# cherubicXN/neat

Measured on AMD Instinct MI355X. Metric: ray-samples/s (train step) on ABC-neat-a, higher is better.
Workload: dtype bf16; 1 GPU; C2: abc-neat-a networks, 1024 rays x 128 samples per GPU, depth samples given, train step = forward + loss + backward + Adam; rays_per_gpu=1024, samples_per_ray=128, global_rays=1024, parallelism=dp1, weights=synthetic 'rough' (seed 42), launch=hip graph replay, the whole step one launch (forward + loss + backward + Adam)

## Files before the change

neat_amd/csrc/kernels_bf16.hpp:

```cpp
#pragma once
#include "kernels.hpp"
#include "bf16_common.hpp"

namespace neat {

__device__ __forceinline__ size_t oct_index(int f, int p, int ldp) { return ((size_t)(f >> 3) * ldp + p) * 8 + (f & 7); }

struct SegH { const void* p; int rows; int bf16; };

struct LayerArgsH {
  SegH in[2];
  int Kpad;
  const uint4* Wp;
  const float* bias;
  int bias_rot, bias_n;
  int N, NT;
  int ldp;
  void* out0; void* out1;
  int out0_bf16, out1_bf16, n_split, accumulate;
  const u16* aux0; const u16* aux1;
  const u16* padfill_oct;
  const float* padfill; int padfill_rows;
};

// ... 753 lines not shown
      eh[3 + 6 * k + c] = f * __cosf(xc * f) * gc;
      eh[6 + 6 * k + c] = -f * __sinf(xc * f) * gc;
      f *= 2.0f;
    }
  }
  eh[39] = 0.0f; ev[39] = 0.0f;
#pragma unroll
  for (int j = 0; j < 39; ++j) { a.Eh[(size_t)j * ldp + p] = eh[j]; ev[j] = a.E[(size_t)j * ldp + p]; }
  auto octet = [](const float (&v)[40], int r0) {
    float t[8];
#pragma unroll
    for (int e = 0; e < 8; ++e) t[e] = (r0 + e < 39) ? v[r0 + e] : 0.0f;
    return make_uint4(pack2(t[0], t[1]), pack2(t[2], t[3]), pack2(t[4], t[5]), pack2(t[6], t[7]));
  };
#pragma unroll
  for (int o = 0; o < 5; ++o) {
    reinterpret_cast<uint4*>(a.Ebf)[(size_t)o * ldp + p] = octet(ev, 8 * o);
    reinterpret_cast<uint4*>(a.Ehbf)[(size_t)o * ldp + p] = octet(eh, 8 * o);
  }
#pragma unroll
  for (int o = 0; o < 4; ++o) {
    reinterpret_cast<uint4*>(a.Ebf4)[(size_t)o * ldp + p] = octet(ev, 7 + 8 * o);
    reinterpret_cast<uint4*>(a.Ehbf4)[(size_t)o * ldp + p] = octet(eh, 7 + 8 * o);
  }
}

#ifndef NEAT_W3_ABLATE
#define NEAT_W3_ABLATE 0
#endif
constexpr int W3T = 512, W3P = 32, W3NS = 4;
template <int NCB> struct W3Cfg {
  static constexpr int QA = 8, QB = 2 * NCB;
  static constexpr int STAGE = (QA + QB) * 2048;
  static constexpr int LDS = W3NS * STAGE;
  static constexpr int QPW = NCB == 5 ? 3 : 2;
  static constexpr int G = 2 * QPW;
};
constexpr int W3_STAGE = W3Cfg<4>::STAGE;
constexpr int W3_LDS_BYTES = W3Cfg<4>::LDS;
constexpr int W3_SLOTS = 12;
struct WgradArgsH3 {
  const unsigned short* A[W3_SLOTS]; const unsigned short* B[W3_SLOTS]; int rowsA[W3_SLOTS];
  const unsigned short* B2[W3_SLOTS];
  int splitB, octsB;
  int npairs, N, K, P, ldp, chunk;
  float* partial; size_t row_stride, split_stride; int col_off, bias_col;
  int nt_loads;
  int interleave;
  int nprob; size_t prob_stride;
};
typedef short v4s16 __attribute__((ext_vector_type(4)));

template <int NCB>
__global__ __launch_bounds__(W3T, 2) void wgrad_kernel_h3(WgradArgsH3 a) {
  typedef W3Cfg<NCB> C;
  extern __shared__ __attribute__((aligned(16))) unsigned char w3lds[];
  typedef __attribute__((address_space(3))) void* lds_ptr;
  typedef __attribute__((address_space(3))) v4s16* lds_v4;
  typedef const __attribute__((address_space(1))) void* gbl_ptr;
  const int tid = threadIdx.x, lane = tid & 63, wave = tid >> 6;
  const int wr = (wave >> 1) * 64, wc = (wave & 1) * 32 * NCB;
  const int nsplit = gridDim.y;
  const int pstep = a.interleave ? nsplit * W3P : W3P;
  const int pbeg = a.interleave ? blockIdx.y * W3P : blockIdx.y * a.chunk;
  const int pend = a.interleave ? a.P : min(a.P, pbeg + a.chunk);
  const int nsteps = a.interleave ? ((a.P + W3P - 1) / W3P - (int)blockIdx.y + nsplit - 1) / nsplit : (pend - pbeg + W3P - 1) / W3P;
  const int prob = a.nprob > 1 ? (int)blockIdx.x : 0;
  const int T = nsteps * a.npairs;
  bool liveR[2], liveC[NCB];
#pragma unroll
  for (int i = 0; i < 2; ++i) liveR[i] = wr + 32 * i < a.N;
#pragma unroll
  for (int j = 0; j < NCB; ++j) liveC[j] = wc + 32 * j < a.K;
  f32x16 acc[2][NCB];
#pragma unroll
  for (int i = 0; i < 2; ++i)
#pragma unroll
    for (int j = 0; j < NCB; ++j)
#pragma unroll
      for (int r = 0; r < 16; ++r) acc[i][j][r] = 0.0f;
  float rsum[2] = {0.0f, 0.0f};

  const int dl_oct = lane & 3, dl_pt = lane >> 2;
  const unsigned lds_base = (unsigned)(size_t)(lds_ptr)w3lds;
  const unsigned short* opbase[2][C::QPW]; const unsigned short* opbase2[2]; int opmax[2][C::QPW]; int opq[C::QPW]; bool opB[C::QPW];
#pragma unroll
  for (int hq = 0; hq < C::QPW; ++hq) {
    const int g = min(C::QPW * wave + hq, C::QA + C::QB - 1);
    opB[hq] = g >= C::QA; opq[hq] = opB[hq] ? g - C::QA : g;
  }
#pragma unroll
  for (int q = 0; q < 2; ++q) {
    const int idx = prob * a.npairs + q;
    const unsigned short* pA = a.A[0]; const unsigned short* pB = a.B[0]; const unsigned short* p2 = a.B2[0];
    int rA = a.rowsA[0];
#pragma unroll
    for (int k = 1; k < W3_SLOTS; ++k)
      if (idx == k) { pA = a.A[k]; pB = a.B[k]; p2 = a.B2[k]; rA = a.rowsA[k]; }
    opbase2[q] = p2;
#pragma unroll
    for (int hq = 0; hq < C::QPW; ++hq) { opbase[q][hq] = opB[hq] ? pB : pA; opmax[q][hq] = opB[hq] ? a.octsB - 1 : (rA + 7) / 8 - 1; }
  }
  auto issue = [&](int tau) {
    const int q = tau >= nsteps ? 1 : 0;
    const int st = tau - q * nsteps;
    if (NEAT_W3_ABLATE == 4) return;
    const unsigned short* base2 = q ? opbase2[1] : opbase2[0];
    const unsigned stage = lds_base + (tau % W3NS) * C::STAGE;
#pragma unroll
    for (int hq = 0; hq < C::QPW; ++hq) {
      const unsigned short* base = q ? opbase[1][hq] : opbase[0][hq];
      const int maxoct = q ? opmax[1][hq] : opmax[0][hq];
      const int oct = min(4 * opq[hq] + dl_oct, maxoct);
      const bool second = opB[hq] && oct >= a.splitB;
      const uint4* seg = reinterpret_cast<const uint4*>(second ? base2 : base) + (size_t)(second ? oct - a.splitB : oct) * a.ldp;
      const int g = min(C::QPW * wave + hq, C::QA + C::QB - 1);
#ifndef NEAT_W3_SKIP_SURPLUS
#define NEAT_W3_SKIP_SURPLUS 1
#endif
      if constexpr (NEAT_W3_SKIP_SURPLUS && 8 * C::QPW > C::QA + C::QB) { if (C::QPW * wave + hq >= C::QA + C::QB) continue; }
// ... 38 lines not shown
        if (NEAT_W3_ABLATE == 2) { av[i] = make_uint4(lane, tau, i, s2); continue; }
        const unsigned char* ap = slot + ((wr >> 5) + i) * 2048 + s2 * 1024 + frag_off;
        const v4s16 lo = __builtin_amdgcn_ds_read_tr16_b64_v4i16((lds_v4)(ap));
        const v4s16 hi = __builtin_amdgcn_ds_read_tr16_b64_v4i16((lds_v4)(ap + 256));
        av[i] = make_uint4(((const unsigned*)&lo)[0], ((const unsigned*)&lo)[1], ((const unsigned*)&hi)[0], ((const unsigned*)&hi)[1]);
      }
#pragma unroll
      for (int j = 0; j < NCB; ++j) {
        if (NEAT_W3_ABLATE == 2) { bv[j] = make_uint4(lane, tau, j, s2); continue; }
        const unsigned char* bp = slot + C::QA * 2048 + ((wc >> 5) + j) * 2048 + s2 * 1024 + frag_off;
        const v4s16 lo = __builtin_amdgcn_ds_read_tr16_b64_v4i16((lds_v4)(bp));
        const v4s16 hi = __builtin_amdgcn_ds_read_tr16_b64_v4i16((lds_v4)(bp + 256));
        bv[j] = make_uint4(((const unsigned*)&lo)[0], ((const unsigned*)&lo)[1], ((const unsigned*)&hi)[0], ((const unsigned*)&hi)[1]);
      }
      if (tail) {
        const int p0 = pb + 16 * s2 + 8 * (G >> 1);
        auto mask4 = [&](uint4& v) {
          unsigned w4[4] = {v.x, v.y, v.z, v.w};
#pragma unroll
          for (int e = 0; e < 4; ++e) {
            const bool k0 = p0 + 2 * e < pend, k1 = p0 + 2 * e + 1 < pend;
            w4[e] = (k0 ? (w4[e] & 0x0000FFFFu) : 0u) | (k1 ? (w4[e] & 0xFFFF0000u) : 0u);
          }
          v = make_uint4(w4[0], w4[1], w4[2], w4[3]);
        };
#pragma unroll
        for (int i = 0; i < 2; ++i) mask4(av[i]);
#pragma unroll
        for (int j = 0; j < NCB; ++j) mask4(bv[j]);
      }
      if (bias_now) {
#pragma unroll
        for (int i = 0; i < 2; ++i) {
          const unsigned w4[4] = {av[i].x, av[i].y, av[i].z, av[i].w};
          float t = rsum[i];
#pragma unroll
          for (int e = 0; e < 4; ++e) { t += bf_lo(w4[e]); t += bf_hi(w4[e]); }
          asm volatile("" : "+v"(t));
          rsum[i] = t;
        }
      }
#pragma unroll
      for (int i = 0; i < 2; ++i) {
        if (!liveR[i]) continue;
#pragma unroll
        for (int j = 0; j < NCB; ++j)
          if (liveC[j]) {
            if (NEAT_W3_ABLATE == 1) { asm volatile("" :: "v"(av[i].x), "v"(av[i].w), "v"(bv[j].x), "v"(bv[j].w)); continue; }
            acc[i][j] = NEAT_MFMA16(*reinterpret_cast<bf16x8*>(&av[i]), *reinterpret_cast<bf16x8*>(&bv[j]), acc[i][j], 0, 0, 0);
          }
      }
    }
  }
  float* dstp = a.partial + (size_t)prob * a.prob_stride + (size_t)blockIdx.y * a.split_stride;
  auto put = [&](float* q, float v) {
    if (NEAT_W3_ABLATE == 3 && v != 123.0f) return;
    *q = v;
  };
#pragma unroll
  for (int i = 0; i < 2; ++i) {
    if (!liveR[i]) continue;
#pragma unroll
    for (int r = 0; r < 16; ++r) {
      const int n = wr + 32 * i + (r & 3) + 8 * (r >> 2) + 4 * (lane >> 5);
      if (n >= a.N) continue;
#pragma unroll
      for (int j = 0; j < NCB; ++j) {
        const int k = wc + 32 * j + (lane & 31);
        if (liveC[j] && k < a.K) put(dstp + (size_t)n * a.row_stride + a.col_off + k, acc[i][j][r]);
      }
    }
  }
  if (do_bias) {
#pragma unroll
    for (int i = 0; i < 2; ++i) {
      float v = rsum[i];
      v += __shfl_xor(v, 32);
      const int n = wr + 32 * i + (lane & 31);
      if (lane < 32 && n < a.N) put(dstp + (size_t)n * a.row_stride + a.bias_col, v);
    }
  }
}

struct PackDesc2 {
  int layer, transpose, N, K, Kpad, NT;
  int s0, s0p, off0, off1;
  int rot;
  float scale; int offset; int blk0; int bf16;
  int lo;
};
constexpr int MAXPACKS2 = 48;
struct PackArgs2 { NetPtrs net; const float* rowscale; int row_off[NLAYERS + 1]; PackDesc2 d[MAXPACKS2]; int npacks; float* out; };

__device__ __forceinline__ float packed_weight(const PackDesc2& d, const float* v, const float* rs, int O, int I, int n, int k) {
  if (!v || n >= d.N || k >= d.K) return 0.0f;
  const int po = d.transpose ? k : n;
  const int pj = d.transpose ? n : k;
  if (po >= O) return 0.0f;
  const int o = (po + d.rot) % O;
  int i;
  if (pj < d.s0p) { if (pj >= d.s0) return 0.0f; i = d.off0 + pj; }
  else { i = d.off1 + (pj - d.s0p); if (pj - d.s0p >= I - d.s0) return 0.0f; }
  if (i >= I) return 0.0f;
  return v[(size_t)o * I + i] * rs[o] * d.scale;
}

__global__ __launch_bounds__(WG) void pack_kernel2(PackArgs2 a) {
  int pk = 0;
  while (pk + 1 < a.npacks && (int)blockIdx.x >= a.d[pk + 1].blk0) ++pk;
  const PackDesc2 d = a.d[pk];
  const int nt = blockIdx.x - d.blk0;
  const int O = a.net.O[d.layer], I = a.net.I[d.layer];
  const float* v = a.net.v[d.layer];
  const float* rs = a.rowscale + a.row_off[d.layer];
  if (d.bf16) {
    const int KS = d.Kpad >> 4;
    uint4* out = reinterpret_cast<uint4*>(a.out + d.offset) + (size_t)nt * KS * 64;
    for (int e = blockIdx.y * WG + threadIdx.x; e < KS * 64; e += WG * gridDim.y) {
      const int s = e >> 6, ln = e & 63;
      const int n = nt * 32 + (ln & 31), kb = 16 * s + 8 * (ln >> 5);
      float w[8];
#pragma unroll
      for (int t = 0; t < 8; ++t) w[t] = packed_weight(d, v, rs, O, I, n, kb + t);
      if (d.lo) {
#pragma unroll
        for (int t = 0; t < 8; ++t) w[t] -= bf2f(f2bf(w[t]));
      }
      out[e] = make_uint4(pack2(w[0], w[1]), pack2(w[2], w[3]), pack2(w[4], w[5]), pack2(w[6], w[7]));
    }
  } else {
    const int KS = d.Kpad >> 1;
    float* out = a.out + d.offset + (size_t)nt * KS * 64;
    for (int e = blockIdx.y * WG + threadIdx.x; e < KS * 64; e += WG * gridDim.y) {
      const int s = e >> 6, ln = e & 63;
// ... 78 lines not shown
```

neat_amd/csrc/neat_net.hip:

```cpp
#include <mutex>
#include <unordered_map>
#if defined(NEAT_HALF) && NEAT_HALF
#define neat neat_f16
#include "f16_symbols.h"
#endif
#include "kernels_bf16.hpp"
#include "kernels_dw.hpp"
#include "fused_launch.hpp"
#include "../../include/neat_hip.h"
#include <algorithm>
#include <initializer_list>
#include <utility>
#include <math.h>
#include <stdio.h>
#include <stdlib.h>
#include <vector>

using namespace neat;

namespace {

constexpr int L_REND = 9, L_ATTR = 14;
const int kO[NLAYERS] = {256, 256, 256, 217, 256, 256, 256, 256, 257, 256, 256, 256, 256, 3, 256, 256, 256, 256, 6};
const int kI[NLAYERS] = {39, 256, 256, 256, 256, 256, 256, 256, 256, 289, 256, 256, 256, 256, 265, 256, 256, 256, 256};
// ... 111 lines not shown
  s->flops = flops; s->bytes = bytes; s->cls = cls;
  hipEventRecord(s->e0, st);
  return s;
}
inline void prof_end(hipStream_t st, ProfSlot* s) { if (s) hipEventRecord(s->e1, st); }

template <int EPI> hipError_t launch_layer_f(hipStream_t st, const LayerArgs& a, int ntiles_p) {
  NEAT_TRY(lds_limit<&layer_kernel<EPI>>(96 * 1024));
  size_t lds = (size_t)a.Kpad * BM * sizeof(float);
  if (a.NT <= 2 && lds < 32768) lds = 32768;
  hipLaunchKernelGGL(layer_kernel<EPI>, dim3(ntiles_p), dim3(WG), lds, st, a);
  return hipGetLastError();
}
int g_wgrad_h3 = 1;
int g_pt_bf16 = 2;

template <int EPI, int PT, bool OBF> hipError_t launch_layer_h_pt(hipStream_t st, const LayerArgsH& a) {
  NEAT_TRY((lds_limit<&layer_kernel_h<EPI, PT, OBF>>(96 * 1024)));
  constexpr int BMT = 32 * PT;
  size_t lds = (size_t)(a.Kpad / 8) * BMT * 16;
  const size_t red = (size_t)4 * PT * 16 * 64 * 4;
  if (a.NT <= 2 && lds < red) lds = red;
  hipLaunchKernelGGL((layer_kernel_h<EPI, PT, OBF>), dim3(a.ldp / BMT), dim3(WG), lds, st, a);
  return hipGetLastError();
}
template <int EPI> hipError_t launch_layer_h(hipStream_t st, const LayerArgsH& a, int) {
  if (a.out0_bf16) return g_pt_bf16 == 4 ? launch_layer_h_pt<EPI, 4, true>(st, a) : launch_layer_h_pt<EPI, 2, true>(st, a);
  return launch_layer_h_pt<EPI, 2, false>(st, a);
}
int g_wgrad_batch = -1;
inline int wgrad_batch_size(int ldp) {
  if (g_wgrad_batch >= 0) return g_wgrad_batch;
  return ldp <= 200000 ? 3 : (ldp <= 400000 ? 2 : 0);
}
int g_wreduce_direct = 2;
int g_head_chain = 2;
int g_fused_adj = 1;
int g_layer_ws = 1;
constexpr int WS_GRID = 256;
constexpr int DW_MAXGRID = 256;
inline int dw_slots(int ldp) {
  const int nt = ldp / WSP;
  return nt < DW_MAXGRID ? (nt > 0 ? nt : 1) : DW_MAXGRID;
}
inline int dw_grid(int ldp) {
  const int nt = ldp / WSP;
  return nt < DW_MAXGRID ? nt : DW_MAXGRID;
}
int g_ws_aux_nt = 15;
int g_ws_wide_store = 1;
const int* g_gate = nullptr; int g_gate_value = 0;
int g_ws_interleave = 1;
int g_wgrad_narrow = 1;
int g_dw_ablate = 0;
int g_dw_fused = 1;
constexpr int DW_MIN_POINTS = 49152;
constexpr int DW8_XBLOCKS = 512;
int g_dw_lin8 = 1;
int g_chain_pp = 1;
constexpr int DW_NSUB = 16;
int g_dw_segments = 1;
template <int EPI, bool FULL> hipError_t launch_layer_wsdw(hipStream_t st, const LayerArgsDW* d0, int n = 1) {
  NEAT_TRY((lds_limit<&layer_kernel_wsdw<EPI, FULL>>(WsCfg<EPI, 16>::LDS + DW_XLDS)));
  if (n < 1 || n > DW_MAXSEG || (n > 1 && !(FULL && EPI != EPI_BWD8))) return hipErrorInvalidValue;
  LayerArgsDWSeg seg{};
  seg.n = n;
  for (int i = 0; i < n; ++i) {
    LayerArgsDW& d = seg.l[i];
    d = d0[i];
    d.w.ntiles = d.w.ldp / WSP;
    d.w.aux_nt = (g_ws_aux_nt & 3) | ((g_ws_aux_nt >> 1) & 28);
    d.ablate = g_dw_ablate;
    if (FULL && (d.w.N != 256 || d.rowsA != 256)) return hipErrorInvalidValue;
    if (d.w.ldp != d0[0].w.ldp) return hipErrorInvalidValue;
  }
  hipLaunchKernelGGL((layer_kernel_wsdw<EPI, FULL>), dim3(dw_grid(seg.l[0].w.ldp)), dim3(WST), (WsCfg<EPI, 16>::LDS + DW_XLDS), st, seg);
  return hipGetLastError();
}
template <int EPI, bool FULL> hipError_t launch_layer_wsdw(hipStream_t st, const LayerArgsDW& d0) { return launch_layer_wsdw<EPI, FULL>(st, &d0, 1); }
template <int EPI, int KS = 16, bool OUTF = false> hipError_t launch_layer_ws(hipStream_t st, const LayerArgsWS& a0) {
  NEAT_TRY((lds_limit<&layer_kernel_ws<EPI, KS, OUTF>>(WsCfg<EPI, KS>::LDS)));
  LayerArgsWS a = a0;
  a.ntiles = a.ldp / WSP;
  a.per_wg = (a.ntiles + WS_GRID - 1) / WS_GRID;
  int grid = (a.ntiles + a.per_wg - 1) / a.per_wg;
  a.tile_stride = 1;
  a.wide_store = g_ws_wide_store;
  a.aux_nt = (g_ws_aux_nt & 3) | ((g_ws_aux_nt >> 1) & 28);
  a.xcd_major = g_ws_interleave == 2;
  if (g_ws_interleave) { grid = a.ntiles < WS_GRID ? a.ntiles : WS_GRID; a.tile_stride = grid; }
  hipLaunchKernelGGL((layer_kernel_ws<EPI, KS, OUTF>), dim3(grid), dim3(WST), (WsCfg<EPI, KS>::LDS), st, a);
  return hipGetLastError();
}
inline int ws_shape(int epi, const LayerArgsH& a) {
  if (!g_layer_ws) return 0;
  const bool seg1 = a.in[1].rows != 0;
  if (!a.in[0].bf16 || a.accumulate || (a.bias && a.bias_rot != 0)) return 0;
  if (a.padfill) {
    return (epi == EPI_TAN && a.padfill_oct && a.padfill_rows == 7 && a.N == 217 && a.Kpad == 256 && !seg1 && a.in[0].rows == 256 &&
            a.out0_bf16 && a.out1 && a.out1_bf16 && a.n_split >= a.N && !a.bias) ? 5 : 0;
  }
  if (a.Kpad == 320) {
    return (epi == EPI_RELU && seg1 && a.in[1].bf16 && a.in[0].rows == 256 && a.in[1].rows <= 64 && a.out0_bf16 && a.N == 256 &&
            a.n_split >= a.N && !a.out1) ? 4 : 0;
  }
  if (a.Kpad == 64 && !seg1) {
// ... 133 lines not shown
    a.out0 = out0.p; a.out1 = out1.p; a.out0_bf16 = out0.bf16; a.out1_bf16 = out1.bf16;
    a.n_split = n_split; a.accumulate = accumulate;
    a.aux0 = reinterpret_cast<const u16*>(aux0.p); a.aux1 = reinterpret_cast<const u16*>(aux1.p);
    a.padfill = padfill; a.padfill_rows = padfill_rows; a.padfill_oct = reinterpret_cast<const u16*>(padfill_oct.p);
    if ((aux0.p && !aux0.bf16) || (aux1.p && !aux1.bf16) || (out1.p && (out1.bf16 != (epi == EPI_TAN)))) return hipErrorInvalidValue;
    const int shape = ws_shape(epi, a);
    e = shape ? dispatch_ws(c.st, epi, a, shape) : dispatch_h(c.st, epi, a, c.ldp / BMH);
  }
  prof_end(c.st, ps);
  dbg_sync(c.st, "layer pid/epi/N", pid, epi, N);
  return e;
}

hipError_t layer_ws(const Ctx& c, int pid, int epi, Arr in0, int N, Arr out0, Arr aux0 = Arr{}, Arr aux1 = Arr{},
                    const float* srow = nullptr, const float* wrow = nullptr, const float* wrow_scale = nullptr,
                    const float* rho_num = nullptr, const float* rho_den = nullptr) {
  const PackDesc2& d = c.L().d[pid];
  if (!c.prec || !in0.bf16 || !out0.bf16 || N > 256 || N > d.N || d.Kpad < 256) return hipErrorInvalidValue;
  LayerArgsWS a{};
  a.in = reinterpret_cast<const u16*>(in0.p); a.Wp = reinterpret_cast<const uint4*>(c.packed + d.offset);
  a.aux0 = reinterpret_cast<const u16*>(aux0.p); a.aux1 = reinterpret_cast<const u16*>(aux1.p);
  a.out0 = reinterpret_cast<u16*>(out0.p);
  a.srow = srow; a.wrow = wrow; a.wrow_scale = wrow_scale; a.rho_num = rho_num; a.rho_den = rho_den;
  a.N = N; a.in_octs = 32; a.ldp = c.ldp; a.kstride = d.Kpad / 16;
  a.split_oct = 32; a.n_split = 1 << 30;
  const double P = (double)c.P;
  const double bytes = 256 * P * 2.0 + N * P * 2.0 * (1 + (aux0.p ? 1 : 0) + (aux1.p ? 1 : 0)) + (srow ? P * 4.0 : 0.0) + N * 256 * 2.0;
  ProfSlot* ps = prof_begin(c.st, 0, 2.0 * N * 256 * P, bytes);
  hipError_t e = dispatch_ws_args(c.st, epi, a);
  prof_end(c.st, ps);
  dbg_sync(c.st, "layer_ws pid/epi/N", pid, epi, N);
  return e;
}

inline dim3 grid1(int n, int b = 256) { return dim3((n + b - 1) / b); }

struct SdfWs {
  float *x, *E, *sdfraw, *sdf, *mask, *g, *e0, *es, *Eh, *gh, *abar8, *ones, *partial;
  Arr featc;
  Arr Ebf, Ebf4, Ehbf, Ehbf4;
  Arr h[9], feat, u[8], vh[9], m[8];
  Arr hlo[9], featlo;
  float *dwp, *dwscale, *dwbias;
  size_t total;
};
constexpr int DW_JOBS = 15;
constexpr int WSPLIT = 128;
constexpr int WLDN = 384, WLDK = 384;
constexpr int W2SPLIT = 256;
constexpr int W2LDN = 288, W2LDK = 320;
constexpr int W2_LDS_BYTES = 2 * 256 * HLD + 8 * 8 * 64 * 16;
constexpr int WGROUPS = 8;
constexpr size_t WSTAGE_FLOATS = (size_t)WGROUPS * WREDUCE_BATCH * 256 * 264;
constexpr size_t WPARTIAL_FLOATS = (size_t)W2SPLIT * W2LDN * W2LDK + WSTAGE_FLOATS;

SdfWs sdf_ws(float* base, int ldp, int mode, int prec, int hx3 = 0) {
  SdfWs w{};
  size_t off = 0;
  auto take = [&](int rows) { float* p = base ? base + off : nullptr; off += (size_t)rows * ldp; return p; };
  auto big = [&](int rows) { Arr a; a.p = take(rows); a.bf16 = prec; return a; };
  w.x = take(3); w.E = take(PE_ROWS + 1); w.sdf = take(1); w.mask = take(1); w.g = take(3); w.sdfraw = take(1);
  if (mode == 0) {
    Arr a = big(256), b = big(256);
    for (int l = 1; l <= 8; ++l) w.h[l] = (l & 1) ? a : b;
  } else if (mode == 2) {
    for (int l = 1; l <= 8; ++l) w.h[l] = big(256);
    if (prec) w.feat = big(256);
    else { float* out8 = take(257); w.sdfraw = out8; w.feat = F(out8 + ldp); }
    Arr a = big(256), b = big(256);
    for (int l = 0; l < 8; ++l) w.u[l] = (l & 1) ? a : b;
    w.e0 = take(PE_ROWS); w.es = take(PE_ROWS);
  } else {
    for (int l = 1; l <= 8; ++l) w.h[l] = big(256);
    if (prec) w.feat = big(256);
    else { float* out8 = take(257); w.sdfraw = out8; w.feat = F(out8 + ldp); }
    for (int l = 0; l < 8; ++l) w.u[l] = big(256);
    w.e0 = take(PE_ROWS); w.es = take(PE_ROWS);
    w.Eh = take(PE_ROWS); w.gh = take(3);
    for (int l = 1; l <= 8; ++l) w.vh[l] = big(256);
    for (int l = 0; l < 8; ++l) w.m[l] = big(256);
    w.abar8 = take(257); w.ones = take(1);
    if (prec) { w.Ebf = big(20); w.Ebf4 = big(16); w.Ehbf = big(20); w.Ehbf4 = big(16); w.featc = big(256); }
    w.partial = base ? base + off : nullptr;
    off += WPARTIAL_FLOATS;
    if (prec) {
      const size_t slots = (size_t)dw_slots(ldp);
      w.dwp = base ? base + off : nullptr; off += (size_t)DW_JOBS * slots * DW_WG_UINT4 * 4;
      w.dwscale = base ? base + off : nullptr; off += (size_t)DW_JOBS * slots * 8;
      w.dwbias = base ? base + off : nullptr; off += (size_t)DW_JOBS * slots * 256;
    }
  }
  if (hx3 && mode != 0) {
    for (int l = 1; l <= 8; ++l) w.hlo[l] = big(128);
    w.featlo = big(128);
  }
  w.total = off;
  return w;
}

struct HeadWs {
  float *small_r, *small_a, *rgb, *lin, *zrgb, *dlin, *sc_r, *sc_a;
  Arr hr[5], ha[5], ar[4], aa[4];
  Arr smallbf_r, smallbf_a, topbf_r, topbf_a;
  float *mr[5], *ma[5];
  size_t total;
};
HeadWs head_ws(float* base, int ldp, int prec, bool fwd_only = false) {
// ... 119 lines not shown
      e = layer(c, L.tr[l], EPI_REV, in(w.u[l], kO[l]), NOIN, nullptr, 256, w.u[l - 1], F(w.es), 217, w.h[l]);
    } else {
      e = layer(c, L.tr[l], EPI_REV, in(w.u[l], kO[l]), NOIN, nullptr, kI[l], w.u[l - 1], Arr{}, 1 << 30, w.h[l]);
    }
    if (e != hipSuccess) return e;
  }
  return layer(c, L.tr[0], EPI_LINEAR, in(w.u[0], 256), NOIN, nullptr, PE_ROWS, F(w.e0));
}

struct WPair { Arr A; int rowsA; int A_rot, A_mod; Arr B[3]; int rowsB[3]; };

struct PackJob { const float* src; int rows; Arr dst; };
void oct_pack(const Ctx& c, std::initializer_list<PackJob> jobs) {
  OctPackArgs a{};
  for (const PackJob& j : jobs) a.job[a.njobs++] = OctPackJob{j.src, j.rows, reinterpret_cast<u16*>(j.dst.p)};
  a.ldp = c.ldp;
  hipLaunchKernelGGL(oct_pack_kernel, dim3((c.ldp + 255) / 256), dim3(256), 0, c.st, a);
}
inline bool oct_operands(const Ctx& c) { return c.prec && g_wgrad_h3; }

void wreduce_layer(const Ctx& c, int layer_id, const neat_net_grads* gr, int K, WreduceArgs& r) {
  const PackDesc2& d = c.L().d[c.L().fwd[layer_id]];
  r.O = kO[layer_id]; r.I = kI[layer_id];
  r.s0 = d.s0; r.s0p = d.s0p; r.off0 = d.off0; r.off1 = d.off1; r.rot = d.rot; r.scale = d.scale;
  r.v = c.net->v[layer_id]; r.g = c.net->g[layer_id];
  r.dv = gr->dv[layer_id]; r.dg = gr->dg[layer_id]; r.db = gr->db[layer_id];
  r.bias_col = K;
}

hipError_t wgrad_reduce(const Ctx& c, const SdfWs& w, int layer_id, WreduceArgs r, int Nred, int N, int K, const neat_net_grads* gr) {
  const int splits = r.splits;
  const float* partial = r.partial;
  const bool direct = c.prec && g_wreduce_direct == 1;
  const bool direct4 = c.prec && g_wreduce_direct == 2 && splits > 2 * WGROUPS && (r.split_stride & 3) == 0 &&
                       r.split_stride / 4 <= WRD_MAXK4;
  if (splits > 2 * WGROUPS && !direct && !direct4) {
    const int Kld = (int)r.split_stride, per = (splits + WGROUPS - 1) / WGROUPS;
    float* stage = w.partial + (WPARTIAL_FLOATS - WSTAGE_FLOATS);
    hipLaunchKernelGGL(wpartial_group_sum_kernel, dim3((Kld / 4 + 127) / 128, WGROUPS, Nred), dim3(128), 0, c.st,
                       partial, splits, Kld / 4, WGROUPS, per, Nred, stage);
    r.partial = stage; r.splits = (splits + per - 1) / per;
    r.row_stride = (size_t)WGROUPS * Kld; r.split_stride = Kld;
  }
  wreduce_layer(c, layer_id, gr, K, r);
  dbg_sync(c.st, "wgrad layer/N/K", layer_id, N, K);
  if (direct4) hipLaunchKernelGGL(wreduce_direct_kernel, dim3(r.O), dim3(WG), 0, c.st, r);
  else if (direct && splits > 2 * WGROUPS) hipLaunchKernelGGL(wreduce_wnorm_kernel<16>, dim3(r.O), dim3(1024), 0, c.st, r);
  else hipLaunchKernelGGL(wreduce_wnorm_kernel<4>, dim3(r.O), dim3(WG), 0, c.st, r);
  dbg_sync(c.st, "wreduce layer/splits", layer_id, splits, 0);
  return hipGetLastError();
}

struct WProb { int layer_id; Arr A[2]; int rowsA[2]; Arr B[2]; };
hipError_t wgrad_multi(const Ctx& c, const SdfWs& w, const WProb* pb, int nprob, int npairs, const neat_net_grads* gr) {
  if (nprob < 2 || npairs < 1 || npairs > 2 || nprob * npairs > W3_SLOTS) return hipErrorInvalidValue;
  for (int p = 0; p < nprob; ++p) if (!gr->dv[pb[p].layer_id]) return hipErrorInvalidValue;
  const int N = 256, K = 256, Kld2 = (K + 1 + 7) / 8 * 8;
  const int per_prob = (W2SPLIT + nprob - 1) / nprob;
  int chunk = ((c.ldp + per_prob - 1) / per_prob + W3P - 1) / W3P * W3P;
  if (chunk < 2 * W3P) chunk = 2 * W3P;
  const int splits = (c.P + chunk - 1) / chunk;
  const size_t region = (size_t)N * splits * Kld2;
  if ((size_t)nprob * region > WPARTIAL_FLOATS - WSTAGE_FLOATS) return hipErrorInvalidValue;
  NEAT_TRY(lds_limit<&wgrad_kernel_h3<4>>(W3_LDS_BYTES));
  WgradArgsH3 a{};
  double flops = 0.0, bytes = 0.0;
  for (int p = 0; p < nprob; ++p)
    for (int q = 0; q < npairs; ++q) {
      if (!pb[p].A[q].bf16 || !pb[p].B[q].bf16 || pb[p].rowsA[q] > 256) return hipErrorInvalidValue;
      const int i = p * npairs + q;
      a.A[i] = reinterpret_cast<const unsigned short*>(pb[p].A[q].p); a.B[i] = reinterpret_cast<const unsigned short*>(pb[p].B[q].p);
      a.B2[i] = nullptr; a.rowsA[i] = pb[p].rowsA[q];
      flops += 2.0 * pb[p].rowsA[q] * 256.0 * (double)c.P;
      bytes += (pb[p].rowsA[q] + 256.0) * (double)c.P * 2.0;
    }
  a.splitB = 32; a.octsB = 32; a.npairs = npairs; a.N = N; a.K = K; a.P = c.P; a.ldp = c.ldp; a.chunk = chunk;
  a.partial = w.partial; a.row_stride = (size_t)splits * Kld2; a.split_stride = Kld2; a.col_off = 0; a.bias_col = K;
  a.nprob = nprob; a.prob_stride = region; a.interleave = g_ws_interleave != 0; a.nt_loads = (g_ws_aux_nt >> 2) & 1;
  ProfSlot* ps = prof_begin(c.st, 1, flops, bytes + (double)nprob * splits * N * (K + 1) * 4.0);
  hipLaunchKernelGGL(wgrad_kernel_h3<4>, dim3(nprob, splits), dim3(W3T), W3_LDS_BYTES, c.st, a);
  prof_end(c.st, ps);
  hipError_t e = hipGetLastError();
  if (splits <= 2 * WGROUPS || nprob > WREDUCE_BATCH) {
    for (int q = 0; q < nprob && e == hipSuccess; ++q) {
      WreduceArgs r{};
      r.partial = w.partial + q * region; r.splits = splits; r.row_stride = (size_t)splits * Kld2; r.split_stride = Kld2;
      e = wgrad_reduce(c, w, pb[q].layer_id, r, N, N, K, gr);
    }
    return e;
  }
  if (e != hipSuccess) return e;
  const bool direct4 = g_wreduce_direct == 2;
  const int per = (splits + WGROUPS - 1) / WGROUPS, groups_used = (splits + per - 1) / per;
  float* stage = w.partial + (WPARTIAL_FLOATS - WSTAGE_FLOATS);
  if (!direct4)
    hipLaunchKernelGGL(wpartial_group_sum_kernel, dim3((Kld2 / 4 + 127) / 128, WGROUPS, nprob * N), dim3(128), 0, c.st,
                       (const float*)w.partial, splits, Kld2 / 4, WGROUPS, per, nprob * N, stage);
  WreduceBatch b{};
  for (int q = 0; q < nprob; ++q) {
    WreduceArgs& r = b.a[q];
    if (direct4) {
      r.partial = w.partial + (size_t)q * region; r.splits = splits; r.row_stride = (size_t)splits * Kld2; r.split_stride = Kld2;
    } else {
      r.partial = stage + (size_t)q * N * WGROUPS * Kld2; r.splits = groups_used;
      r.row_stride = (size_t)WGROUPS * Kld2; r.split_stride = Kld2;
    }
    wreduce_layer(c, pb[q].layer_id, gr, K, r);
  }
  if (direct4) hipLaunchKernelGGL(wreduce_direct_batch_kernel, dim3(256, nprob), dim3(WG), 0, c.st, b);
  else hipLaunchKernelGGL(wreduce_wnorm_batch_kernel, dim3(256, nprob), dim3(WG), 0, c.st, b);
  return hipGetLastError();
}

struct RowDot { const float* s; Arr B0, B1; };

hipError_t wgrad(const Ctx& c, const SdfWs& w, int layer_id, const WPair* pairs_in, int npairs, int N, const neat_net_grads* gr,
                 const RowDot* rd = nullptr) {
  if (!gr->dv[layer_id]) return hipSuccess;
  const PackDesc2& d = c.L().d[c.L().fwd[layer_id]];
  const int K = d.s0p + (kI[layer_id] - d.s0);
  double wflops = 0.0;
  for (int q = 0; q < npairs; ++q)
    wflops += 2.0 * pairs_in[q].rowsA * (pairs_in[q].rowsB[0] + pairs_in[q].rowsB[1] + pairs_in[q].rowsB[2]) * (double)c.P;
  double wbytes = 0.0;
  for (int q = 0; q < npairs; ++q) {
    wbytes += pairs_in[q].rowsA * (double)c.P * (pairs_in[q].A.bf16 ? 2.0 : 4.0);
    for (int t = 0; t < 3; ++t) wbytes += pairs_in[q].rowsB[t] * (double)c.P * (pairs_in[q].B[t].bf16 ? 2.0 : 4.0);
  }
  WreduceArgs r{};
  int splits, chunk_used = 0;
  if (!c.prec) {
    WPair pairs[2] = {pairs_in[0], npairs > 1 ? pairs_in[1] : WPair{}};
    for (int s = 0; s < 3; ++s)
      if (pairs[0].rowsB[s] == 0) { pairs[0].B[s] = F(w.ones); pairs[0].rowsB[s] = 1; break; }
    const int Kt = K + 1;
    int chunk = ((c.ldp + WSPLIT - 1) / WSPLIT + WBP - 1) / WBP * WBP;
    if (chunk < 2 * WBP) chunk = 2 * WBP;
    splits = (c.P + chunk - 1) / chunk;
    const int ntile = (N + 127) / 128, ktiles = (Kt + 127) / 128;
    WgradArgs a{};
    for (int q = 0; q < npairs; ++q) {
      a.pair[q].A = pairs[q].A.f(); a.pair[q].rowsA = pairs[q].rowsA;
      for (int s = 0; s < 3; ++s) { a.pair[q].B[s] = pairs[q].B[s].f(); a.pair[q].rowsB[s] = pairs[q].rowsB[s]; }
    }
    a.npairs = npairs; a.N = N; a.Kt = Kt; a.P = c.P; a.ldp = c.ldp; a.chunk = chunk;
    a.partial = w.partial; a.row_stride = (size_t)splits * WLDK; a.split_stride = WLDK; a.ktiles = ktiles; a.x3 = c.x3;
    ProfSlot* ps = prof_begin(c.st, 1, wflops, wbytes + (double)splits * N * Kt * 4.0);
    hipLaunchKernelGGL(wgrad_kernel, dim3(ntile * ktiles, splits), dim3(WG), 0, c.st, a);
    prof_end(c.st, ps);
    r.row_stride = (size_t)splits * WLDK; r.split_stride = WLDK;
  } else {
    NEAT_TRY(lds_limit<&wgrad_kernel_h2>(W2_LDS_BYTES));
    const int Kld2 = (K + 1 + 7) / 8 * 8;
    if (Kld2 > W2LDK) return hipErrorInvalidValue;
    bool h3 = g_wgrad_h3 && N <= 256;
    for (int q = 0; q < npairs && h3; ++q) {
      const WPair& s = pairs_in[q];
      h3 = s.A.bf16 && s.A_mod == 0 && s.rowsA <= 256 && s.B[0].bf16 && s.rowsB[2] == 0 &&
           (s.rowsB[1] == 0 || (s.B[1].bf16 && s.rowsB[0] % 8 == 0)) &&
           s.rowsB[0] == pairs_in[0].rowsB[0] && s.rowsB[1] == pairs_in[0].rowsB[1];
    }
    const int r0 = pairs_in[0].rowsB[0], r1 = pairs_in[0].rowsB[1];
// ... 338 lines not shown
      a.nvalid = ((n_main < 0 ? c.P : n_main) + 63) / 64;
      a.feat = reinterpret_cast<const u16*>(feat.p);
      a.smallbf = reinterpret_cast<const u16*>((head ? h.smallbf_a : h.smallbf_r).p); a.srows = head ? SMALL_A : SMALL_R;
      for (int l = 0; l < 5; ++l) {
        a.Wp[l] = reinterpret_cast<const uint4*>(c.packed + L.d[L.fwd[base + l]].offset);
        a.bias[l] = c.net->b[base + l];
        a.hid[l] = (l && save) ? reinterpret_cast<u16*>(hh[l].p) : nullptr;
        a.mask[l] = (l && save) ? reinterpret_cast<u16*>(head ? h.ma[l] : h.mr[l]) : nullptr;
      }
      if (L.d[L.fwd[base]].Kpad != 320 || L.d[L.fwd[base + 4]].Kpad != 256) return hipErrorInvalidValue;
      a.out = head ? h.lin : h.rgb;
      double fl = 0.0;
      for (int l = 0; l < 5; ++l) fl += 2.0 * kO[base + l] * kI[base + l] * (double)c.P;
      ProfSlot* ps = prof_begin(c.st, 4, fl, (double)c.P * (512.0 + a.srows * 2.0 + (save ? 4 * (512.0 + 64.0) : 0.0) + (head ? 24.0 : 12.0)) + 2.0 * 540000.0);
      e = launch_head_chain(c.st, a, head, c.ldp / 64, WS_GRID, save);
      prof_end(c.st, ps);
      if (e != hipSuccess) return e;
    }
    return hipSuccess;
  }
  for (int head = 0; head < 2; ++head) {
    const int base = head ? L_ATTR : L_REND;
    const Arr* hh = head ? h.ha : h.hr;
    const float* small = head ? h.small_a : h.small_r;
    const int srows = head ? SMALL_A : SMALL_R;
    const In small_in = c.prec ? in(head ? h.smallbf_a : h.smallbf_r, srows) : in(F(small), srows);
    if ((e = layer(c, L.fwd[base], EPI_RELU, in(feat, 256), small_in, c.net->b[base], 256, hh[1])) != hipSuccess) return e;
    for (int l = 1; l < 4; ++l)
      if ((e = layer(c, L.fwd[base + l], EPI_RELU, in(hh[l], 256), NOIN, c.net->b[base + l], 256, hh[l + 1])) != hipSuccess) return e;
    if (head == 0) e = layer(c, L.fwd[base + 4], EPI_SIGMOID, in(hh[4], 256), NOIN, c.net->b[base + 4], 3, F(h.rgb));
    else e = layer(c, L.fwd[base + 4], EPI_LINEAR, in(hh[4], 256), NOIN, c.net->b[base + 4], 6, F(h.lin));
    if (e != hipSuccess) return e;
  }
  return hipSuccess;
}

hipError_t heads_backward(const Ctx& c, const HeadWs& h, const SdfWs& w, const neat_net_grads* gr, const float* slot = nullptr,
                          const float* slot_a = nullptr, int n_main = -1) {
  const PackLayout& L = c.L();
  hipError_t e;
  const bool oct = oct_operands(c);
  const int nb1 = wgrad_batch_size(c.ldp);
  const bool batch = oct && nb1 && g_wgrad_h3;
  bool wdone[2] = {false, false};
  auto head_wgrads = [&](int head, bool per_head_batch) -> hipError_t {
    const int base = head ? L_ATTR : L_REND;
    const Arr* hh = head ? h.ha : h.hr;
    const Arr* ab = head ? h.aa : h.ar;
    const float* top = head ? h.dlin : h.zrgb;
    const float* small = head ? h.small_a : h.small_r;
    const int srows = head ? SMALL_A : SMALL_R;
    hipError_t e2;
    const bool hb = per_head_batch && batch;
    if (hb) {
      WProb pb[4];
      for (int l = 1; l <= 3; ++l) pb[l - 1] = WProb{base + l, {ab[l], Arr{}}, {256, 0}, {hh[l], Arr{}}};
      pb[3] = WProb{base + 4, {head ? h.topbf_a : h.topbf_r, Arr{}}, {kO[base + 4], 0}, {hh[4], Arr{}}};
      if ((e2 = wgrad_multi(c, w, pb, 4, 1, gr)) != hipSuccess) return e2;
    }
    for (int l = 0; l <= 4; ++l) {
      if ((hb || (!per_head_batch && batch)) && l >= 1 && l <= 3) continue;
      if (l == 4 && hb) continue;
      WPair pr[1] = {};
      pr[0].A = l == 4 ? (oct ? (head ? h.topbf_a : h.topbf_r) : F(top)) : ab[l]; pr[0].rowsA = kO[base + l];
      if (l == 0) {
        pr[0].B[0] = w.feat; pr[0].rowsB[0] = 256;
        pr[0].B[1] = oct ? (head ? h.smallbf_a : h.smallbf_r) : F(small); pr[0].rowsB[1] = srows;
      } else {
        pr[0].B[0] = hh[l]; pr[0].rowsB[0] = 256;
      }
      if ((e2 = wgrad(c, w, base + l, pr, 1, kO[base + l], gr)) != hipSuccess) return e2;
    }
    wdone[head] = true;
    return hipSuccess;
  };
  for (int head = 0; head < 2; ++head) {
    const int base = head ? L_ATTR : L_REND;
    const Arr* hh = head ? h.ha : h.hr;
    const Arr* ab = head ? h.aa : h.ar;
    const float* top = head ? h.dlin : h.zrgb;
    const int top_rows = head ? 6 : 3;
    const float* small = head ? h.small_a : h.small_r;
    const int srows = head ? SMALL_A : SMALL_R;
    if (oct && g_head_chain == 2 && head_masks_written(h)) {
      HeadBwdArgs a{};
      a.P = c.P; a.ldp = c.ldp;
      a.nvalid = ((n_main < 0 ? c.P : n_main) + 63) / 64;
      a.top = reinterpret_cast<const u16*>((head ? h.topbf_a : h.topbf_r).p);
      for (int l = 0; l < 5; ++l) {
        a.Wt[l] = reinterpret_cast<const uint4*>(c.packed + L.d[L.tr[base + l]].offset);
        a.mask[l] = l ? reinterpret_cast<const u16*>(head ? h.ma[l] : h.mr[l]) : nullptr;
      }
      for (int l = 0; l < 4; ++l) a.ab[l] = reinterpret_cast<u16*>(ab[l].p);
      if (L.d[L.tr[base + 4]].Kpad != 64 || L.d[L.tr[base]].Kpad != 256) return hipErrorInvalidValue;
      a.featc = reinterpret_cast<u16*>(w.featc.p);
      a.accumulate = head;
      a.rho_num = (head && slot_a) ? slot : nullptr; a.rho_den = (head && slot_a) ? slot_a : nullptr;
      a.sc = head ? h.sc_a : h.sc_r; a.srows = srows;
      double fl = 0.0;
      for (int l = 0; l < 5; ++l) fl += 2.0 * kO[base + l] * kI[base + l] * (double)c.P;
      ProfSlot* ps = prof_begin(c.st, 4, fl, (double)c.P * (16.0 + 4 * (512.0 + 64.0) + (head ? 1024.0 : 512.0) + srows * 4.0) + 2.0 * 540000.0);
      e = launch_head_bwd_chain(c.st, a, head, c.ldp / 64, WS_GRID);
      prof_end(c.st, ps);
      if (e != hipSuccess) return e;
      if ((!batch || nb1 >= 3) && (e = head_wgrads(head, true)) != hipSuccess) return e;
      continue;
    }
    if ((e = layer(c, L.tr[base + 4], EPI_BWD_RELU, in(oct ? (head ? h.topbf_a : h.topbf_r) : F(top), top_rows), NOIN, nullptr, 256, ab[3], Arr{}, 1 << 30, hh[4])) != hipSuccess) return e;
    for (int l = 3; l >= 1; --l)
      if ((e = layer(c, L.tr[base + l], EPI_BWD_RELU, in(ab[l], 256), NOIN, nullptr, 256, ab[l - 1], Arr{}, 1 << 30, hh[l])) != hipSuccess) return e;
    if (c.prec) {
      if ((e = layer_ws(c, L.tr[base], head ? EPI_LINACC : EPI_LINEAR, ab[0], 256, w.featc, head ? w.featc : Arr{}, Arr{}, nullptr, nullptr, nullptr,
                        (head && slot_a) ? slot : nullptr, (head && slot_a) ? slot_a : nullptr)) != hipSuccess) return e;
      if ((e = layer(c, L.tr[base], EPI_LINEAR, in(ab[0], 256), NOIN, nullptr, srows, F(head ? h.sc_a : h.sc_r), Arr{}, 1 << 30,
                     Arr{}, Arr{}, 0, 0, 1 << 30, nullptr, 0, 8)) != hipSuccess) return e;
// ... 144 lines not shown
      hipLaunchKernelGGL(export_out8_kernel, dim3((P + 255) / 256, 32), dim3(256), 0, c.st, (const float*)w.sdfraw, reinterpret_cast<const u16*>(w.feat.p),
                         reinterpret_cast<const u16*>(w.featlo.p), P, c.ldp, out257, feat);
  } else {
    if (out257) hipLaunchKernelGGL(fm_to_rm_kernel, grid1(P), dim3(256), 0, c.st, w.sdfraw, P, 257, c.ldp, out257, 0);
    if (feat) hipLaunchKernelGGL(fm_to_rm_kernel, grid1(P), dim3(256), 0, c.st, w.feat.f(), P, 256, c.ldp, feat, 0);
  }
}

Ctx make_ctx(const Prec& pr, const float* packed, const neat_net_params* net, int P, void* stream) {
  Ctx c{(hipStream_t)stream, packed, net, P, round_ldp(P, pr.prec), pr.prec};
  c.x3 = pr.x3; c.hx3 = pr.hx3;
  return c;
}

}

#if !NEAT_HALF
#define NEAT_TWIN(fn) extern "C" decltype(fn) f16_##fn;
#include "twin_list.h"
#undef NEAT_TWIN
__attribute__((visibility("hidden"))) int neat_aux_set_tuning(int key, int value);
#define NEAT_F16_FWD(call) if (precision == 3) { precision = BF16; return f16_##call; } if (precision == HX3 || precision == HX3_FASTVALUES) return f16_##call;
#else
#define NEAT_F16_FWD(call)
#endif

extern "C" {

#if !NEAT_HALF
int neat_abi_version(void) { return 15; }
#endif

int neat_set_tuning(int key, int value) {
#if !NEAT_HALF
  if (key == 28 || key == 30) return neat_aux_set_tuning(key, value);
  f16_neat_set_tuning(key, value);
#endif
  if (key == 0 && (value == 2 || value == 4)) { g_pt_bf16 = value; return 0; }
  if (key == 1 && (value == 0 || value == 1)) { g_wgrad_h3 = value; return 0; }
  if (key == 2 && (value == 0 || value == 1)) { g_layer_ws = value; return 0; }
  if (key == 6 && value >= 0 && value <= 2) { g_wreduce_direct = value; return 0; }
  if (key == 8 && (value == -1 || value == 0 || value == 2 || value == 3 || value == 6)) { g_wgrad_batch = value; return 0; }
  if (key == 9 && value >= 0 && value <= 2) { g_ws_interleave = value; return 0; }
  if (key == 11 && value >= 0 && value <= 63) { g_ws_aux_nt = value; return 0; }
  if (key == 12 && (value == 0 || value == 1)) { g_ws_wide_store = value; return 0; }
  if (key == 13 && (value == 0 || value == 1)) { g_fused_adj = value; return 0; }
  if (key == 14 && value >= 0 && value <= 2) { g_head_chain = value; return 0; }
  if (key == 16 && value >= 0 && value <= 2) { g_dw_fused = value; return 0; }
  if (key == 17 && value >= 0 && value <= 7) { g_dw_ablate = value; return 0; }
  if (key == 21 && value >= 0 && value <= 4) { g_wgrad_narrow = value; return 0; }
  if (key == 22 && (value == 0 || value == 1)) { g_dw_lin8 = value; return 0; }
  if (key == 24 && (value == 0 || value == 1)) { g_chain_pp = value; return 0; }
  if (key == 25 && (value == 0 || value == 1)) { g_dw_segments = value; return 0; }
  return -1;
}

int neat_prof_enable(int on) {
#if !NEAT_HALF
  f16_neat_prof_enable(on);
#endif
  g_prof.on = on != 0;
  g_prof.used = 0;
  return 0;
}

int neat_prof_collect(int cls, double* total_ms, double* total_flops, int* launches, double* total_bytes) {
  double ms = 0.0, fl = 0.0, by = 0.0;
  int n = 0;
  for (size_t i = 0; i < g_prof.used; ++i) {
    ProfSlot& s = g_prof.pool[i];
    if (s.cls != cls) continue;
    hipError_t e = hipEventSynchronize(s.e1);
    if (e != hipSuccess) return (int)e;
    float t = 0.0f;
    if ((e = hipEventElapsedTime(&t, s.e0, s.e1)) != hipSuccess) return (int)e;
    ms += t; fl += s.flops; by += s.bytes; ++n;
  }
#if !NEAT_HALF
  {
    double ms2 = 0.0, fl2 = 0.0, by2 = 0.0;
    int n2 = 0;
    const int rc = f16_neat_prof_collect(cls, &ms2, &fl2, &n2, &by2);
    if (rc != 0) return rc;
    ms += ms2; fl += fl2; by += by2; n += n2;
  }
#endif
  if (total_ms) *total_ms = ms;
  if (total_flops) *total_flops = fl;
  if (launches) *launches = n;
  if (total_bytes) *total_bytes = by;
  return 0;
}

size_t neat_packed_floats(int precision) {
  NEAT_F16_FWD(neat_packed_floats(precision))
  const Prec pr = resolve(precision);
  return (!pr.ok || pr.hx3 == 2) ? 0 : pack_layout(pr.prec, pr.hx3 != 0).total;
}

int neat_pack_weights(const neat_net_params* net, float* packed, int precision, void* stream) {
  NEAT_F16_FWD(neat_pack_weights(net, packed, precision, stream))
  const Prec pr = resolve(precision);
  if (pr.hx3 == 2) return -1;
  if (!net || !packed || !pr.ok) return -1;
  hipStream_t st = (hipStream_t)stream;
  const PackLayout& L = pack_layout(pr.prec, pr.hx3 != 0);
// ... 280 lines not shown
```

Before: 49.60 million ray-samples/s.

## Fuse the head's wide layer-0 weight gradient into the batched wgrad launch

Folds the head's first-layer weight-gradient GEMM (K = 256 + small rows, 5 column blocks) into the same kernel launch as the four batched 256x256 head wgrads, using a block-index dispatch between two instantiations of a shared body. Its split partials go into an enlarged partial buffer and are reduced in the same batched reduce launch as the others. This removes a separate wgrad launch and a separate reduction per head and fills the grid with more blocks. In exchange the workspace grows, and the mixed NCB=4/5 blocks share one LDS size and launch bound, which may lower occupancy for the narrower problems.

```diff
diff --git a/neat_amd/csrc/kernels_bf16.hpp b/neat_amd/csrc/kernels_bf16.hpp
--- a/neat_amd/csrc/kernels_bf16.hpp
+++ b/neat_amd/csrc/kernels_bf16.hpp
@@ -829,7 +829,7 @@
 typedef short v4s16 __attribute__((ext_vector_type(4)));
 
 template <int NCB>
-__global__ __launch_bounds__(W3T, 2) void wgrad_kernel_h3(WgradArgsH3 a) {
+__device__ __forceinline__ void wgrad_h3_body(const WgradArgsH3& a, const int prob, const int ysplit, const int nsplit) {
   typedef W3Cfg<NCB> C;
   extern __shared__ __attribute__((aligned(16))) unsigned char w3lds[];
   typedef __attribute__((address_space(3))) void* lds_ptr;
@@ -837,12 +837,10 @@
   typedef const __attribute__((address_space(1))) void* gbl_ptr;
   const int tid = threadIdx.x, lane = tid & 63, wave = tid >> 6;
   const int wr = (wave >> 1) * 64, wc = (wave & 1) * 32 * NCB;
-  const int nsplit = gridDim.y;
   const int pstep = a.interleave ? nsplit * W3P : W3P;
-  const int pbeg = a.interleave ? blockIdx.y * W3P : blockIdx.y * a.chunk;
+  const int pbeg = a.interleave ? ysplit * W3P : ysplit * a.chunk;
   const int pend = a.interleave ? a.P : min(a.P, pbeg + a.chunk);
-  const int nsteps = a.interleave ? ((a.P + W3P - 1) / W3P - (int)blockIdx.y + nsplit - 1) / nsplit : (pend - pbeg + W3P - 1) / W3P;
-  const int prob = a.nprob > 1 ? (int)blockIdx.x : 0;
+  const int nsteps = a.interleave ? ((a.P + W3P - 1) / W3P - ysplit + nsplit - 1) / nsplit : (pend - pbeg + W3P - 1) / W3P;
   const int T = nsteps * a.npairs;
   bool liveR[2], liveC[NCB];
 #pragma unroll
@@ -987,7 +985,7 @@
       }
     }
   }
-  float* dstp = a.partial + (size_t)prob * a.prob_stride + (size_t)blockIdx.y * a.split_stride;
+  float* dstp = a.partial + (size_t)prob * a.prob_stride + (size_t)ysplit * a.split_stride;
   auto put = [&](float* q, float v) {
     if (NEAT_W3_ABLATE == 3 && v != 123.0f) return;
     *q = v;
@@ -1015,6 +1013,15 @@
       if (lane < 32 && n < a.N) put(dstp + (size_t)n * a.row_stride + a.bias_col, v);
     }
   }
+}
+template <int NCB>
+__global__ __launch_bounds__(W3T, 2) void wgrad_kernel_h3(WgradArgsH3 a) {
+  wgrad_h3_body<NCB>(a, a.nprob > 1 ? (int)blockIdx.x : 0, (int)blockIdx.y, (int)gridDim.y);
+}
+__global__ __launch_bounds__(W3T, 2) void wgrad_kernel_h3_head(WgradArgsH3 a, WgradArgsH3 b, int nsplit_a) {
+  const int na = a.nprob * nsplit_a, x = (int)blockIdx.x;
+  if (x < na) wgrad_h3_body<4>(a, x % a.nprob, x / a.nprob, nsplit_a);
+  else wgrad_h3_body<5>(b, 0, x - na, (int)gridDim.x - na);
 }
 
 struct PackDesc2 {
diff --git a/neat_amd/csrc/neat_net.hip b/neat_amd/csrc/neat_net.hip
--- a/neat_amd/csrc/neat_net.hip
+++ b/neat_amd/csrc/neat_net.hip
@@ -187,6 +187,7 @@
 const int* g_gate = nullptr; int g_gate_value = 0;
 int g_ws_interleave = 1;
 int g_wgrad_narrow = 1;
+int g_wgrad_head5 = 1;
 int g_dw_ablate = 0;
 int g_dw_fused = 1;
 constexpr int DW_MIN_POINTS = 49152;
@@ -426,7 +427,9 @@
 constexpr int W2_LDS_BYTES = 2 * 256 * HLD + 8 * 8 * 64 * 16;
 constexpr int WGROUPS = 8;
 constexpr size_t WSTAGE_FLOATS = (size_t)WGROUPS * WREDUCE_BATCH * 256 * 264;
-constexpr size_t WPARTIAL_FLOATS = (size_t)W2SPLIT * W2LDN * W2LDK + WSTAGE_FLOATS;
+constexpr size_t WHEAD5_FLOATS = (size_t)4 * 256 * 64 * 264 + (size_t)W2SPLIT * 256 * W2LDK;
+constexpr size_t WPARTIAL_FLOATS = WHEAD5_FLOATS + WSTAGE_FLOATS;
+static_assert(WHEAD5_FLOATS >= (size_t)W2SPLIT * W2LDN * W2LDK, "partial tiles of the widest single layer");
 
 SdfWs sdf_ws(float* base, int ldp, int mode, int prec, int hx3 = 0) {
   SdfWs w{};
@@ -652,8 +655,20 @@
 }
 
 struct WProb { int layer_id; Arr A[2]; int rowsA[2]; Arr B[2]; };
-hipError_t wgrad_multi(const Ctx& c, const SdfWs& w, const WProb* pb, int nprob, int npairs, const neat_net_grads* gr) {
+struct WWide { int layer_id; Arr A; int rowsA; Arr B, B2; int rowsB2; };
+struct W3Split { int chunk, splits; };
+inline W3Split w3_split(const Ctx& c, int target) {
+  int chunk = ((c.ldp + target - 1) / target + W3P - 1) / W3P * W3P;
+  if (chunk < 2 * W3P) chunk = 2 * W3P;
+  return W3Split{chunk, (c.P + chunk - 1) / chunk};
+}
+inline bool wgrad_head5_fits(const Ctx& c) {
+  return g_wgrad_head5 && g_wgrad_h3 && g_wreduce_direct == 2 && w3_split(c, (W2SPLIT + 3) / 4).splits > 2 * WGROUPS &&
+         w3_split(c, W2SPLIT).splits > 2 * WGROUPS;
+}
+hipError_t wgrad_multi(const Ctx& c, const SdfWs& w, const WProb* pb, int nprob, int npairs, const neat_net_grads* gr, const WWide* wide = nullptr) {
   if (nprob < 2 || npairs < 1 || npairs > 2 || nprob * npairs > W3_SLOTS) return hipErrorInvalidValue;
+  if (wide && (nprob != 4 || npairs != 1 || !wgrad_head5_fits(c) || !gr->dv[wide->layer_id])) return hipErrorInvalidValue;
   for (int p = 0; p < nprob; ++p) if (!gr->dv[pb[p].layer_id]) return hipErrorInvalidValue;
   const int N = 256, K = 256, Kld2 = (K + 1 + 7) / 8 * 8;
   const int per_prob = (W2SPLIT + nprob - 1) / nprob;
@@ -677,9 +692,36 @@
   a.splitB = 32; a.octsB = 32; a.npairs = npairs; a.N = N; a.K = K; a.P = c.P; a.ldp = c.ldp; a.chunk = chunk;
   a.partial = w.partial; a.row_stride = (size_t)splits * Kld2; a.split_stride = Kld2; a.col_off = 0; a.bias_col = K;
   a.nprob = nprob; a.prob_stride = region; a.interleave = g_ws_interleave != 0; a.nt_loads = (g_ws_aux_nt >> 2) & 1;
-  ProfSlot* ps = prof_begin(c.st, 1, flops, bytes + (double)nprob * splits * N * (K + 1) * 4.0);
-  hipLaunchKernelGGL(wgrad_kernel_h3<4>, dim3(nprob, splits), dim3(W3T), W3_LDS_BYTES, c.st, a);
-  prof_end(c.st, ps);
+  bytes += (double)nprob * splits * N * (K + 1) * 4.0;
+  WreduceArgs rw{};
+  int Kw = 0;
+  if (wide) {
+    const PackDesc2& d = c.L().d[c.L().fwd[wide->layer_id]];
+    Kw = d.s0p + (kI[wide->layer_id] - d.s0);
+    const int Kldw = (Kw + 1 + 7) / 8 * 8;
+    const W3Split sw = w3_split(c, W2SPLIT);
+    if (!wide->A.bf16 || !wide->B.bf16 || !wide->B2.bf16 || wide->rowsA > 256 || wide->rowsB2 < 1 || wide->rowsB2 > 64 ||
+        Kw != 256 + wide->rowsB2 || Kldw > W2LDK || Kldw / 4 > WRD_MAXK4) return hipErrorInvalidValue;
+    float* partw = w.partial + (size_t)nprob * region;
+    if ((size_t)nprob * region + (size_t)N * sw.splits * Kldw > WPARTIAL_FLOATS - WSTAGE_FLOATS) return hipErrorInvalidValue;
+    NEAT_TRY(lds_limit<&wgrad_kernel_h3_head>(W3Cfg<5>::LDS));
+    WgradArgsH3 b{};
+    b.A[0] = reinterpret_cast<const unsigned short*>(wide->A.p); b.B[0] = reinterpret_cast<const unsigned short*>(wide->B.p);
+    b.B2[0] = reinterpret_cast<const unsigned short*>(wide->B2.p); b.rowsA[0] = wide->rowsA;
+    b.K = Kw; b.splitB = 32; b.octsB = (Kw + 7) / 8; b.col_off = 0; b.bias_col = Kw;
+    b.npairs = 1; b.N = N; b.P = c.P; b.ldp = c.ldp; b.chunk = sw.chunk;
+    b.partial = partw; b.row_stride = (size_t)sw.splits * Kldw; b.split_stride = Kldw; b.interleave = a.interleave; b.nt_loads = a.nt_loads;
+    flops += 2.0 * wide->rowsA * (double)Kw * (double)c.P;
+    bytes += (wide->rowsA + (double)Kw) * (double)c.P * 2.0 + (double)sw.splits * N * (Kw + 1) * 4.0;
+    ProfSlot* ps = prof_begin(c.st, 1, flops, bytes);
+    hipLaunchKernelGGL(wgrad_kernel_h3_head, dim3(nprob * splits + sw.splits), dim3(W3T), W3Cfg<5>::LDS, c.st, a, b, splits);
+    prof_end(c.st, ps);
+    rw.partial = partw; rw.splits = sw.splits; rw.row_stride = b.row_stride; rw.split_stride = Kldw;
+  } else {
+    ProfSlot* ps = prof_begin(c.st, 1, flops, bytes);
+    hipLaunchKernelGGL(wgrad_kernel_h3<4>, dim3(nprob, splits), dim3(W3T), W3_LDS_BYTES, c.st, a);
+    prof_end(c.st, ps);
+  }
   hipError_t e = hipGetLastError();
   if (splits <= 2 * WGROUPS || nprob > WREDUCE_BATCH) {
     for (int q = 0; q < nprob && e == hipSuccess; ++q) {
@@ -707,7 +749,11 @@
     }
     wreduce_layer(c, pb[q].layer_id, gr, K, r);
   }
-  if (direct4) hipLaunchKernelGGL(wreduce_direct_batch_kernel, dim3(256, nprob), dim3(WG), 0, c.st, b);
+  if (wide) {
+    b.a[nprob] = rw;
+    wreduce_layer(c, wide->layer_id, gr, Kw, b.a[nprob]);
+  }
+  if (direct4) hipLaunchKernelGGL(wreduce_direct_batch_kernel, dim3(256, nprob + (wide ? 1 : 0)), dim3(WG), 0, c.st, b);
   else hipLaunchKernelGGL(wreduce_wnorm_batch_kernel, dim3(256, nprob), dim3(WG), 0, c.st, b);
   return hipGetLastError();
 }
@@ -1152,15 +1198,19 @@
     const int srows = head ? SMALL_A : SMALL_R;
     hipError_t e2;
     const bool hb = per_head_batch && batch;
+    bool five = false;
     if (hb) {
       WProb pb[4];
       for (int l = 1; l <= 3; ++l) pb[l - 1] = WProb{base + l, {ab[l], Arr{}}, {256, 0}, {hh[l], Arr{}}};
       pb[3] = WProb{base + 4, {head ? h.topbf_a : h.topbf_r, Arr{}}, {kO[base + 4], 0}, {hh[4], Arr{}}};
-      if ((e2 = wgrad_multi(c, w, pb, 4, 1, gr)) != hipSuccess) return e2;
+      const WWide wd{base, ab[0], kO[base], w.feat, head ? h.smallbf_a : h.smallbf_r, srows};
+      five = wgrad_head5_fits(c) && gr->dv[base] != nullptr;
+      if ((e2 = wgrad_multi(c, w, pb, 4, 1, gr, five ? &wd : nullptr)) != hipSuccess) return e2;
     }
     for (int l = 0; l <= 4; ++l) {
       if ((hb || (!per_head_batch && batch)) && l >= 1 && l <= 3) continue;
       if (l == 4 && hb) continue;
+      if (l == 0 && five) continue;
       WPair pr[1] = {};
       pr[0].A = l == 4 ? (oct ? (head ? h.topbf_a : h.topbf_r) : F(top)) : ab[l]; pr[0].rowsA = kO[base + l];
       if (l == 0) {
@@ -1411,6 +1461,7 @@
   if (key == 22 && (value == 0 || value == 1)) { g_dw_lin8 = value; return 0; }
   if (key == 24 && (value == 0 || value == 1)) { g_chain_pp = value; return 0; }
   if (key == 25 && (value == 0 || value == 1)) { g_dw_segments = value; return 0; }
+  if (key == 26 && (value == 0 || value == 1)) { g_wgrad_head5 = value; return 0; }
   return -1;
 }
 
```

Result: no change. 49.90 million ray-samples/s, median of 6 (+0.6%).
